# ubc-vision/UniT

Measured on AMD Instinct MI355X. Metric: images/sec (fwd+bwd+SGD) R101-C4 VOC 600x1000 bs=2/GPU, higher is better.
Workload: dtype bf16; 1 GPU; UniT base-training step S1 (TrainerNoMeta.run_step): ResNet-101-C4, VOC split1 K=20, 2 supervised + 2 weak 3x600x1000 images per GPU, 512 RoIs/image, two Res5 heads, RPN 12000->2000, all 8 losses, SGD momentum; images_per_gpu=2, global_batch=2, parallelism=dp1

## Files before the change

include/unit_hip.h:

```cpp
#ifndef UNIT_HIP_H
#define UNIT_HIP_H
#include <stddef.h>
#include <stdint.h>
#ifdef __cplusplus
extern "C" {
#endif

int unit_version(void);
const char* unit_build_hash(void);
const char* unit_last_error(void);

int unit_preprocess_image(const float* img_chw, int C, int H, int W, const float* mean3, const float* std3, float prescale,
                          void* out_nhwc, int out_dtype, int Hmax, int Wmax, int Cpad, void* stream);
int unit_resize_u8_pass(const unsigned char* src, int H, int W, int C, int axis, const int* bounds, const int* kk, int ksize,
                        int out_size, unsigned char* dst, void* stream);
int unit_preprocess_u8(const unsigned char* img_hwc, int C, int H, int W, int hflip, const float* mean3, const float* std3,
                       float prescale, void* out_nhwc, int out_dtype, int Hmax, int Wmax, int Cpad, void* stream);
int unit_image_chw_to_u8(const void* img_chw, int src_u8, int C, int H, int W, unsigned char* out_hwc, void* stream);
int unit_tta_boxes(const float* props, const int* count, int P, int Pcap, const float* views, int V, float* out, void* stream);
int unit_nchw_to_nhwc(const float* x, void* y, int dtype, int N, int C, int H, int W, int Cp, void* stream);
int unit_nhwc_to_nchw(const void* x, int dtype, float* y, int N, int C, int H, int W, int Cp, void* stream);
int unit_debug_spin(long long cycles, void* sink, void* stream);
int unit_cast(const void* x, int in_dtype, void* y, int out_dtype, long n, void* stream);
int unit_fill_zero(void* p, size_t nbytes, void* stream);
int unit_add_cast(const float* a32, const void* b, const void* mask_ref, void* y, int dtype, long n, void* stream);

int unit_conv2d_fwd(const void* x, const void* w, void* y, const float* bias, const void* residual, const void* mask_ref,
                    int in_dtype, int out_dtype, int N, int H, int W, int C, int K, int R, int S, int stride, int pad, int OH,
                    int OW, int ldy, int oy_mul, int OHf, int OWf, int relu, int tile_cfg, void* stream);
int unit_conv2d_fwd_big(const void* x, const void* w, void* y, const float* bias, const void* residual, const void* mask_ref,
                        int out_dtype, int N, int H, int W, int C, int K, int R, int S, int stride, int pad, int OH, int OW, int ldy,
                        int oy_mul, int OHf, int OWf, int relu, int variant, void* stream);
size_t unit_conv_pool_partial_floats(int M, int ldy);
size_t unit_relu_bits_bytes(int M, int ldy);
int unit_conv2d_fwd_big_ex(const void* x, const void* w, void* y, const float* bias, const void* residual, const unsigned char* mask_bits,
                           unsigned char* relu_bits, float* pool_partial, int pool_rows, int N, int H, int W, int C, int K, int R, int S,
                           int pad, int ldy, int relu, const void* x2, int C2, int variant, void* stream);
int unit_pool_finish(const float* partial, int R, int rows, int ldy, int K, void* out, int ldo, int out_dtype, void* stream);
int unit_avgpool_bwd_bits(const void* dfeat, const unsigned char* bits, int R, int roi_offset, int rows, int C, void* g, void* stream);
int unit_conv2d_fwd_mid(const void* x, const void* w, void* y, const float* bias, const void* residual, const void* mask_ref,
                        int out_dtype, int N, int H, int W, int C, int K, int R, int S, int stride, int pad, int OH, int OW, int ldy,
                        int oy_mul, int OHf, int OWf, int relu, int tile, void* stream);
int unit_x3_split(const float* x, void* out, long rows, int C, void* stream);
int unit_x3_merge(const void* in, float* out, long rows, int C, void* stream);
int unit_weight_prep_x3(const float* w_krsc, const float* scale_k, int K, int R, int S, int C, void* w_fwd, void* w_dgrad, void* stream);
int unit_conv2d_fwd_x3(const void* x, const void* w, void* y, const float* bias, const void* residual, const void* mask_ref, int mask_c,
                       int N, int H, int W, int C, int K, int R, int S, int stride, int pad, int OH, int OW, int ldy, int oy_mul, int OHf,
                       int OWf, int relu, int tile, void* stream);
int unit_weight_prep_x3s(const float* w_krsc, const float* scale_k, int K, int R, int S, int C, void* w_fwd, void* w_dgrad, int dgrad_segs,
                         void* stream);
int unit_conv2d_fwd_x3s(const void* x, const void* w, void* y, const float* bias, const void* residual, const void* mask_ref, int mask_c,
                        int N, int H, int W, int C, int K, int R, int S, int stride, int pad, int OH, int OW, int ldy, int oy_mul, int OHf,
                        int OWf, int relu, int tile, int segs, void* stream);
int unit_conv2d_wgrad_x3(const void* x, const void* dy, float* dw, const float* scale_k, int N, int H, int W, int C, int K, int R, int S,
                         int stride, int pad, int OH, int OW, int ldy, int accumulate, int variant, void* workspace, size_t workspace_bytes,
                         void* stream);
int unit_global_avgpool_x3_fwd(const void* y, float* out, int R, int rows, int C, void* stream);
int unit_global_avgpool_x3_bwd_relu(const float* dfeat, const void* y, void* g, int R, int rows, int C, void* stream);
typedef struct UnitConvSecond {
  const void* x; void* y; const void* residual; const void* mask_ref;
  int N, H, W, OHf, OWf;
} UnitConvSecond;
int unit_conv2d_fwd_pair(int kernel, const void* x, const void* w, void* y, const float* bias, const void* residual, const void* mask_ref, int mask_c,
                         int in_dtype, int out_dtype, int N, int H, int W, int C, int K, int R, int S, int stride, int pad, int OH, int OW, int ldy,
                         int oy_mul, int OHf, int OWf, int relu, int tile, const UnitConvSecond* second, void* stream);
size_t unit_conv2d_wgrad_workspace_bytes(int in_dtype, int N, int OH, int OW, int K, int R, int S, int C);
int unit_conv2d_wgrad(const void* x, const void* dy, float* dw, const float* scale_k, int in_dtype, int N, int H, int W, int C,
                      int K, int R, int S, int stride, int pad, int OH, int OW, int ldy, int accumulate, int variant, void* workspace,
                      size_t workspace_bytes, void* stream);
int unit_conv2d_wgrad_splits(int in_dtype, int N, int OH, int OW, int K, int R, int S, int C);
typedef struct UnitWgradProblem {
  const void* x; const void* dy; void* partial;
  int N, H, W, C, K, R, S, stride, pad, OH, OW, ldy;
  int splits, kind;
  int x_pitch;
  int x_back, dy_back;
} UnitWgradProblem;
size_t unit_wgrad_problem_bytes(void);
int unit_conv2d_wgrad_group_supported(int in_dtype, int N, int OH, int OW, int K, int R, int S, int C);
int unit_conv2d_wgrad_group_plan(UnitWgradProblem* pr, int n, int splits_hint);
int unit_conv2d_wgrad_group(const UnitWgradProblem* pr, int n, int in_dtype, void* stream);
int unit_conv2d_wgrad_group_layout(const UnitWgradProblem* pr, int n, int* layout, int layout_rows, int* rows);
int unit_wgrad256_loop(void);
int unit_stream_wait_stream(void* waiter, void* signaller);
size_t unit_tensor_desc_bytes(void);
int unit_multi_wgrad_reduce(const void* descs_dev, int n, int total_blocks, float* grads_flat, void* stream);
int unit_multi_weight_prep(const void* descs_dev, int n, int total_blocks, const float* params_flat, int dtype, void* stream);
int unit_shard_sum(const void* parts, int dtype, int nparts, long n, float* out, void* stream);
int unit_comm_unique_id(void* id, int id_bytes);
int unit_comm_init(int rank, int world, const void* id, int id_bytes, void** comm);
int unit_allreduce_bucket_async(void* comm, void* buf, long count, int dtype, void* stream);
int unit_comm_wait(void* compute_stream, void* comm_stream);
int unit_comm_destroy(void* comm);
int unit_comm_rccl_version(void);
int unit_frozen_bn_fold(const float* w, const float* b, const float* rm, const float* rv, float eps, float* scale, float* shift,
                        int C, void* stream);
int unit_weight_prep(const float* w_krsc, const float* scale_k, int K, int R, int S, int C, int Cp, void* w_fwd, void* w_dgrad,
                     int dtype, void* stream);
size_t unit_bias_grad_scratch_bytes(int M, int K);
int unit_bias_grad(const void* dy, int dtype, int M, int K, int ld, float* db, int accumulate, float* scratch, size_t scratch_bytes,
                   void* stream);
size_t unit_linear_wgrad_workspace_bytes(int R, int C, int K);
int unit_linear_wgrad(const void* x, const void* dy, int dtype, int R, int C, int K, int ldy, float* dw, float* db,
                      void* workspace, size_t workspace_bytes, void* stream);
int unit_stem_conv_pool(const void* x, const void* w, const float* shift, void* y, int dtype, int N, int H, int W, void* stream);
int unit_maxpool3x3s2_fwd(const void* x, void* y, int dtype, int N, int H, int W, int C, void* stream);
int unit_global_avgpool_fwd(const void* x, void* y, int dtype, int R, int P, int C, void* stream);
int unit_global_avgpool_bwd_relu(const void* dfeat, const void* out, void* g, int dtype, int R, int P, int C, void* stream);

int unit_anchor_grid(float* out, int H, int W, int A, float stride, float offset, const float* cell_dev, void* stream);

size_t unit_iou_match_workspace_bytes(int B, int Mcap);
int unit_iou_match(const float* gt, const int* gt_count, int B, int Mcap, const float* boxes, long box_batch_stride,
                   const int* box_count, int Ncap, const float* thresholds, const int* labels, int n_thresh,
                   int allow_low_quality, int64_t* match_idx, int8_t* match_label, float* match_val, void* workspace,
                   size_t workspace_bytes, void* stream);
int unit_pairwise_iou(const float* b1, int M, const float* b2, int Nb, float* out, void* stream);
int unit_match_matrix(const float* q, int M, int N, const float* thresholds, const int* labels, int n_thresh, int allow_low_quality,
                      int64_t* match_idx, int8_t* match_label, float* match_val, float* rowmax_ws, void* stream);

int unit_subsample_labels(const void* labels, int labels_are_int64, const int* count, int B, int Ncap, const int* perm, int Pcap,
                          int num_samples, int max_pos, int bg_label, int8_t* out_labels, int* sampled_idx, int* out_counts,
                          void* stream);

int unit_box_encode(const float* src, const float* tgt, const float* weights4, float* out, int n, void* stream);
int unit_box_decode(const float* deltas, int ld, int col0, int K, const float* boxes, const float* weights4, float scale_clamp,
                    float* out, int n, void* stream);

size_t unit_sort_workspace_bytes(int B, int n);
int unit_sort_desc_stable(const float* src, long batch_stride, int ld, int A, int col0, int B, int n, float* out_keys, int* out_idx,
                          void* workspace, size_t workspace_bytes, void* stream);
int unit_sort_desc_stable_topk(const float* src, long batch_stride, int ld, int A, int col0, int B, int n, int topk,
                               float min_exclusive, float* out_keys, int* out_idx, void* workspace, size_t workspace_bytes,
                               void* stream);
int unit_rpn_decode_select(const float* head, long head_batch_stride, int ld, int A, int delta_col0, const float* anchors,
                           const int* sorted_idx, const float* sorted_logit, int B, int Ncap, int topk, const float* image_hw_dev,
                           float scale_clamp, float min_size, float* cand_boxes, float* cand_scores, int* cand_count, void* stream);
size_t unit_nms_workspace_bytes(int B, int cap);
int unit_nms_max_candidates(void);
int unit_nms(const float* boxes_sorted, const float* scores_sorted, const int* count, int B, int cap, float thresh, int max_keep,
             int* keep_idx, int* keep_count, float* out_boxes, float* out_scores, void* workspace, size_t workspace_bytes,
             void* stream);

int unit_append_gt(const float* props, const int* pcount, int Pcap, const float* gt, const int* gcount, int Mcap, int B, float* cat,
                   int* ccount, void* stream);
int unit_roi_classes(const int64_t* match_idx, const int8_t* match_label, const int* count, const int64_t* gt_classes,
                     const int* gcount, int Mcap, int B, int Ncap, int K, int64_t* cls, void* stream);
int unit_gather_rois(const float* cat, int Ncap, const int* sampled_idx, int S, const int64_t* cls, const int64_t* match_idx,
                     const float* gt, const int* gcount, int Mcap, int B, float* rois, int* roi_cls, float* roi_gt, void* stream);
int unit_first_k_rois(const float* props, const int* pcount, int Pcap, int S, int B, int batch_index_offset, float* rois, int* valid,
                      void* stream);

int unit_roi_align_fwd(const void* feat_nhwc, int dtype, int N, int H, int W, int C, const float* rois, const int* roi_count_dev,
                       int R, int pooled_size, int out_size, int bin_step, float spatial_scale, int sampling_ratio, int aligned,
                       void* out, void* stream);
int unit_roi_align_bwd(const void* gout, int dtype, int N, int H, int W, int C, const float* rois, const int* roi_count_dev, int R,
                       int pooled_size, int out_size, int bin_step, float spatial_scale, int sampling_ratio, int aligned,
                       float* dfeat_f32, void* stream);

size_t unit_roi_align_bwd_gather_workspace_bytes(int R);
int unit_roi_align_bwd_gather(const void* gout, int dtype, int N, int H, int W, int C, const float* rois, const int* roi_count_dev,
                              int R, int rois_per_image, int image_offset, int pooled_size, int out_size, int bin_step,
                              float spatial_scale, int sampling_ratio, int aligned, const void* addend, int addend_images,
                              const void* mask_ref, void* dfeat, int out_dtype, void* workspace, size_t workspace_bytes,
                              void* stream);

size_t unit_rpn_loss_scratch_bytes(int B, int Ncap);
int unit_rpn_loss(const float* head, int ld, int A, int dcol0, const int8_t* labels, const int64_t* match_idx, const float* gt_boxes,
                  int Mcap, const float* anchors, int B, int Ncap, float normalizer, float gscale, float* loss2, void* dhead,
                  int dhead_dtype, float* scratch, size_t scratch_bytes, void* stream);
int unit_rpn_loss_w(const float* head, int ld, int A, int dcol0, const int8_t* labels, const int64_t* match_idx, const float* gt_boxes,
                    int Mcap, const float* anchors, int B, int Ncap, float normalizer, float gscale, float w_cls, float w_loc, float* loss2,
                    void* dhead, int dhead_dtype, float* scratch, size_t scratch_bytes, void* stream);
#define UNIT_BOXLOSS_SMOOTH_L1 0
#define UNIT_BOXLOSS_GIOU 1
int unit_rpn_loss_ex(const float* head, int ld, int A, int dcol0, const int8_t* labels, const int64_t* match_idx, const float* gt_boxes,
                     int Mcap, const float* anchors, int B, int Ncap, float normalizer, float gscale, float w_cls, float w_loc, float* loss2,
                     void* dhead, int dhead_dtype, float* scratch, size_t scratch_bytes, int loss_type, float beta, void* stream);
int unit_sup_scores(const float* delta, int ldd, int dcol0, const float* weak, int ldw, int wcol0, int n_oicr, int ncls,
                    const unsigned char* novel_mask_dev, const float* extra, int lde, int ecol0, float* out, int ldo, int R,
                    void* stream);
int unit_softmax_ce(const float* logits, int ld, int col0, int ncls, const int* labels, const float* weights, int R, float gscale,
                    float* loss, void* dy, int dy_dtype, int ldd, int dcol0, unsigned long long* acc, void* stream);
int unit_box_reg_loss(const float* bbox, int ld, int col0, int K, const int* labels, const float* rois5, const float* gt_boxes,
                      const float* weights4, int R, float gscale, float* loss, void* dy, int dy_dtype, int ldd, int dcol0,
                      unsigned long long* acc, void* stream);
int unit_box_reg_loss_ex(const float* bbox, int ld, int col0, int K, const int* labels, const float* rois5, const float* gt_boxes,
                         const float* weights4, int R, float gscale, float* loss, void* dy, int dy_dtype, int ldd, int dcol0,
                         unsigned long long* acc, int loss_type, float beta, void* stream);
int unit_wsddn_mil(const float* streams, int ld, int ccol0, int dcol0, int K, const int* valid, int S, int B,
                   const unsigned char* multihot, float cls_temp, float det_temp, float mil_multiplier, float gscale, float* loss,
                   float* xr_out, void* dy, int dy_dtype, int ldd, int dyc0, int dyd0, void* stream);
int unit_oicr_targets(const float* src, int ld, int col0, int mode, int K, const float* rois5, const int* valid, int S, int B,
                      const unsigned char* multihot, float fg_thresh, float bg_thresh, int* labels, float* weights, void* stream);
int unit_oicr_targets_ex(const float* src, int ld, int col0, int mode, int K, const float* rois5, const int* valid, int S, int B,
                         const unsigned char* multihot, float fg_thresh, float bg_thresh, int* labels, float* weights, float* gt_boxes,
                         void* stream);
int unit_softmax_mean(const float* logits, int ld, int col0, int step, int n, int K, const int* valid, float* out, int ldo, int R,
                      void* stream);
int unit_sum_losses(const float* losses, int n, float* out, void* stream);
int unit_pcl_loss(const float* logits, int ld, int col0, int K, const int* valid, int S, int B, const int* labels, const float* cls_weights,
                  const int* gt_assign, const int* pc_count, const float* pc_img_cls_weights, const float* pc_probs, const int* n_pc,
                  int ldc, float gscale, float* loss, void* dy, int dy_dtype, int ldd, int dcol0, unsigned long long* acc, void* stream);
size_t unit_workspace_bytes_pcl_targets(int B, int S, int n_streams);
int unit_kmeans_draws(unsigned long long* bits7);
int unit_pcl_targets(const float* src, int ld, int col0, int mode, int step, const float* nxt, int ldn, int ncol0, int nmode, int nstep, int K,
                     const float* rois5, const int* valid, int S, int B, int n_streams, const unsigned char* multihot, float fg_thresh,
                     float bg_thresh, float graph_iou_thresh, int max_pc_num, int* labels, float* cls_weights, int* gt_assign, int* n_pc,
                     int* pc_labels, int* pc_count, float* pc_img_cls_weights, float* pc_probs, int ldc, void* workspace,
                     size_t workspace_bytes, void* stream);
int unit_pcl_targets_ex(const float* src, int ld, int col0, int mode, int step, const float* nxt, int ldn, int ncol0, int nmode, int nstep,
                        int K, const float* rois5, const int* valid, int S, int B, int n_streams, const unsigned char* multihot,
                        float fg_thresh, float bg_thresh, float graph_iou_thresh, int max_pc_num, int* labels, float* cls_weights,
                        int* gt_assign, int* n_pc, int* pc_labels, int* pc_count, float* pc_img_cls_weights, float* pc_probs, int ldc,
                        float* gt_boxes, void* workspace, size_t workspace_bytes, void* stream);
int unit_perm_keys(unsigned long long seed, const long long* counter_dev, int stream_id, int B, int n, float* keys, void* stream);
int unit_counter_bump(long long* counter_dev, long long delta, void* stream);

int unit_embedding_similarity(const float* emb, int ld, int dim, const int* novel_rows, int n_novel, const int* base_rows, int n_base,
                              float* out, void* stream);
int unit_similarity(const float* lin_weak, int ld, int col0, int n_oicr, int ncls, const int* base_dev, int n_base, const float* lingual,
                    int n_novel, float visual_threshold, int use_lingual, int use_visual, float* sim, int R, void* stream);
int unit_transfer_predictions(const float* lin, int ld, int ccol0, int bcol0, int K, const float* weak, int ldw, int wcol0, int n_oicr,
                              const float* ft, int ldf, int fccol0, int fbcol0, const float* sim_cls, const float* sim_bbox,
                              const int* base_dev, int n_base, const int* novel_dev, int n_novel, const int8_t* role_dev,
                              const int* slot_dev, float* scores, int lds, float* bbox, int ldb, int R, void* stream);
int unit_transfer_predictions_ex(const float* lin, int ld, int ccol0, int bcol0, int K, const float* weak, int ldw, int wcol0, int n_oicr,
                                 int wbcol0, const float* ft, int ldf, int fccol0, int fbcol0, const float* sim_cls, const float* sim_bbox,
                                 const int* base_dev, int n_base, const int* novel_dev, int n_novel, const int8_t* role_dev,
                                 const int* slot_dev, float* scores, int lds, float* bbox, int ldb, int R, void* stream);
int unit_transfer_predictions_bwd(const void* dy, int dy_dtype, int ldd, int dccol0, int dbcol0, const float* lin, int ld, int ccol0,
                                  int bcol0, int K, const float* sim_cls, const float* sim_bbox, const int* base_dev, int n_base,
                                  const int* novel_dev, int n_novel, const int8_t* role_dev, const int* slot_dev, void* dlin, int ldl,
                                  float* dsim, int R, void* stream);
int unit_similarity_bwd(const float* lin_weak, int ld, int col0, int n_oicr, int ncls, const int* base_dev, int n_base,
                        const float* lingual, int n_novel, float visual_threshold, int use_lingual, int use_visual, const float* dsim,
                        void* dlin, int dlin_dtype, int ldl, int dcol0, int R, void* stream);
int unit_similarity_static(const float* w_master, int ld, int row0, int n_oicr, int ncls, int D, const int* base_dev, int n_base,
                           const int* novel_dev, int n_novel, const float* lingual, float weight, int use_lingual, int k_topk, int k_wtopk,
                           int k_lsda, float* A, void* stream);
int unit_similarity_ex(const float* lin_weak, int ld, int col0, int n_oicr, int ncls, const int* base_dev, int n_base, const float* A,
                       int n_novel, float visual_threshold, float weight, int use_visual, int k_visual, int average, int none, int product,
                       float* sim, int R, void* stream);
int unit_similarity_bwd_ex(const float* lin_weak, int ld, int col0, int n_oicr, int ncls, const int* base_dev, int n_base, const float* A,
                           int n_novel, float visual_threshold, float weight, int use_visual, int k_visual, int average, int none,
                           int product, const float* dsim, void* dlin, int dlin_dtype, int ldl, int dcol0, int R, void* stream);
int unit_softmax_rows(const float* x, int ld, int ncls, float* y, int ldy, int R, void* stream);
int unit_tta_accumulate(const float* scores, int lds, int scol0, const float* deltas, int ldd, long view_rows, int n_in, int K, int R,
                        const int* count, int v, int n, float* probs_sum, float* delta_sum, float* delta_mean, void* stream);
int unit_detection_candidates(const float* probs, int ldp, const float* deltas, int ldd, const float* props, const int* pcount, int B,
                              int Rcap, int K, const float* weights4, float scale_clamp, const float* image_hw_dev, float score_thresh,
                              int cap, float* cand_boxes, float* cand_scores, int* cand_class, int* cand_roi, int* cand_count,
                              float* cand_max, void* stream);
int unit_detection_offset_gather(const float* cand_boxes, const int* cand_class, const int* order, const int* cand_count,
                                 const float* cand_max, int B, int cap, float* out, void* stream);
int unit_detection_finalize(const float* cand_boxes, const float* cand_scores, const int* cand_class, const int* cand_roi, const int* order,
                            const int* keep, const int* keep_count, int B, int cap, int topk, float* out_boxes, float* out_scores,
                            int* out_class, int* out_roi, int* out_count, void* stream);
int unit_detector_postprocess(float* boxes, const int* count, int B, int topk, const float* scale_xy_dev, const float* out_hw_dev,
                              unsigned char* nonempty, void* stream);
int unit_compact_detections(const float* boxes, const float* scores, const int* cls, const int* roi, const float* masks, int mask_elems,
                            const int* count, const unsigned char* nonempty, int B, int topk, float* oboxes, float* oscores, long* ocls,
                            int* oroi, float* omasks, int* out_count, void* stream);
int unit_boxes_to_rois5(const float* boxes, int B, int T, float* rois5, void* stream);
int unit_gather_rows(const void* src, const int* idx, int B, int T, int rcap, int row_bytes, void* out, void* stream);
int unit_gather_blocks(const void* src, int nb, int block_rows, int take, int row_bytes, void* out, void* stream);
int unit_pseudo_gt(const float* boxes, const float* scores, const int* cls, const int* count, const unsigned char* multihot, int B, int T, int K,
                   float threshold, float* gt_boxes, int* gt_count, int* kept_idx, void* stream);
int unit_gate_anchor_labels(signed char* labels, const int* gt_count, int B, int Ncap, void* stream);

int unit_deconv2x2_weight_prep(const float* w, int Cin, int Cout, void* w_fwd, void* w_dgrad, int dtype, void* stream);
int unit_deconv2x2_grad_unpack(const float* dw_gemm, const float* db_gemm, int Cin, int Cout, float* dw, float* db, void* stream);
int unit_mask_targets(const unsigned char* gt_masks, int Mcap, int Hm, int Wm, const float* rois5, const int* gt_index, const int* cls,
                      int K, int S, int M, unsigned char* out, void* stream);
int unit_mask_targets_polygon(const double* poly_xy, const int* poly_start, const int* inst_start, const int* image_inst0,
                              const float* rois5, const int* gt_index, const int* cls, int K, int S, int M, unsigned char* out, void* stream);
int unit_mask_bce_loss(const float* logits, int K, int ldk, const int* cls, const unsigned char* targets, int S, int M, float gscale,
                       float* loss, void* dlogits, int d_dtype, void* stream);
int unit_mask_bce_loss_ft(const float* logits, int K, int ldk, int delta_col0, const int* cls, const unsigned char* targets,
                          const float* sim, const int* sim_rows, const int* base_dev, int n_base, int n_novel, const int8_t* role_dev,
                          const int* slot_dev, int S, int M, float gscale, float* loss, void* dlogits, int d_dtype, float* dsim,
                          void* stream);
int unit_mask_probs(const float* logits, int K, int ldk, int delta_col0, const int* cls, const float* sim, const int* base_dev, int n_base,
                    int n_novel, const int8_t* role_dev, const int* slot_dev, int S, int M, float* out, void* stream);
int unit_gather_match_index(const int* sampled_idx, int S, const int64_t* match_idx, int Ncap, int B, int* out, void* stream);
int unit_paste_masks(const float* probs, const float* boxes, const unsigned char* valid, int S, int M, int H, int W, float threshold,
                     unsigned char* out, void* stream);

int unit_metrics_rpn(const int8_t* labels, int n, int* m, void* stream);
int unit_metrics_fastrcnn(const float* scores, int ld, int col0, int ncls, const int* roi_cls, int R, int* m, void* stream);
int unit_metrics_mask(const float* logits, int K, int ldk, const int* cls, const unsigned char* targets, int S, int M, int* m, void* stream);

int unit_sgd_momentum(float* p, const float* g, float* buf, long n, float lr, float momentum, float wd, float grad_scale,
                      int first_step, const float* lr_dev, void* stream);

int unit_grad_clip_chunk(void);
size_t unit_grad_clip_workspace_bytes(long g_numel, int n_seg);
int unit_grad_clip_coefs(const float* g, long g_numel, const long* table, int n_seg, int seg_lo, int seg_hi, int n_chunks, int norm_kind,
                         float clip_value, float grad_scale, int full_model, float* norms, float* coefs, void* workspace,
                         size_t workspace_bytes, void* stream);
int unit_sgd_step(float* p, const float* g, float* buf, long lo, long n, float lr, float momentum, float wd, float grad_scale,
                  float clip_value, int first_step, int nesterov, int clip_mode, const long* table, int n_seg, const float* coefs,
                  const float* lr_dev, void* stream);
int unit_sgd_step_masked(float* p, const float* g, float* buf, long lo, long n, float lr, float momentum, float wd, float grad_scale,
                         float clip_value, int first_step, int nesterov, int clip_mode, const long* table, int n_seg, const float* coefs,
                         const unsigned char* live, const float* lr_dev, void* stream);

size_t unit_call_bytes(void);
int unit_replay(const void* calls, int n, int* failed);
int unit_event_record_raw(void* event, void* stream);
int unit_stream_wait_event_raw(void* stream, void* event);
int unit_replay_selftest(int a0, const void* p1, float f0, long a2, int a3, float f1, int a4, int a5, size_t a6, int a7, int a8, float f2,
                         int a9, int a10, int a11, int a12, int a13, int a14, int a15, int a16, int a17, int a18, int a19, int a20,
                         int a21, int a22, int a23, int a24, int a25, int a26, float f3, int a27, long long* out);

#ifdef __cplusplus
}
#endif
#endif
```

unit_amd/csrc/roi_align.hip:

```cpp
#include "common.h"
#include <stdlib.h>

__device__ __forceinline__ long xcd_contiguous(long bid, long n) {
  long q = n / 8, r = n % 8, xcd = bid % 8, loc = bid / 8;
  return (xcd < r ? xcd * (q + 1) : r * (q + 1) + (xcd - r) * q) + loc;
}

struct RoiGeom {
  float sw, sh, bw, bh, count;
  int gh, gw, b;
};

__device__ __forceinline__ RoiGeom roi_geom(const float* __restrict__ roi, float scale, int pooled, int sampling_ratio, bool aligned) {
  RoiGeom g;
  g.b = (int)roi[0];
  float offset = aligned ? 0.5f : 0.0f;
  g.sw = roi[1] * scale - offset; g.sh = roi[2] * scale - offset;
  float ew = roi[3] * scale - offset, eh = roi[4] * scale - offset;
  float rw = ew - g.sw, rh = eh - g.sh;
  if (!aligned) { rw = fmaxf(rw, 1.0f); rh = fmaxf(rh, 1.0f); }
  g.bh = rh / (float)pooled; g.bw = rw / (float)pooled;
  g.gh = sampling_ratio > 0 ? sampling_ratio : (int)ceilf(rh / (float)pooled);
  g.gw = sampling_ratio > 0 ? sampling_ratio : (int)ceilf(rw / (float)pooled);
  g.count = (float)(g.gh * g.gw > 1 ? g.gh * g.gw : 1);
  return g;
}

struct Taps { float w1, w2, w3, w4; int yl, xl, yh, xh; bool valid; };

__device__ __forceinline__ Taps bilinear_taps(float y, float x, int H, int W) {
  Taps t;
  t.valid = !(y < -1.0f || y > (float)H || x < -1.0f || x > (float)W);
  if (y <= 0.f) y = 0.f;
  if (x <= 0.f) x = 0.f;
  int yl = (int)y, xl = (int)x, yh, xh;
  if (yl >= H - 1) { yh = yl = H - 1; y = (float)yl; } else { yh = yl + 1; }
  if (xl >= W - 1) { xh = xl = W - 1; x = (float)xl; } else { xh = xl + 1; }
  float ly = y - (float)yl, lx = x - (float)xl;
  float hy = 1.0f - ly, hx = 1.0f - lx;
  t.w1 = hy * hx; t.w2 = hy * lx; t.w3 = ly * hx; t.w4 = ly * lx;
  t.yl = yl; t.xl = xl; t.yh = yh; t.xh = xh;
  return t;
}

template <typename T, int SR>
__global__ void roi_align_fwd_kernel(const T* __restrict__ feat, int H, int W, int C, const float* __restrict__ rois,
                                     const int* __restrict__ roi_count, int pooled, int out_size, int bin_step, float scale,
                                     int sampling_ratio, int aligned, T* __restrict__ out) {
  int bin = (int)xcd_contiguous(blockIdx.x, gridDim.x);
  int r = bin / (out_size * out_size);
  int pp = bin - r * out_size * out_size;
  int oph = pp / out_size, opw = pp - oph * out_size;
  int c0 = threadIdx.x * 8;
  if (c0 >= C) return;
  T* o = out + ((size_t)bin) * C + c0;
  float acc[8] = {0, 0, 0, 0, 0, 0, 0, 0};
  if (roi_count && r >= *roi_count) { Vec8<T>::store(o, acc); return; }
  RoiGeom g = roi_geom(rois + 5 * (size_t)r, scale, pooled, sampling_ratio, aligned != 0);
  int ph = oph * bin_step, pw = opw * bin_step;
  const T* f = feat + (size_t)g.b * H * W * C + c0;
  if constexpr (SR > 0) {
    Taps t[SR * SR];
    float v[SR * SR][4][8];
#pragma unroll
    for (int iy = 0; iy < SR; ++iy) {
      float y = g.sh + (float)ph * g.bh + ((float)iy + 0.5f) * g.bh / (float)SR;
#pragma unroll
      for (int ix = 0; ix < SR; ++ix) {
        float x = g.sw + (float)pw * g.bw + ((float)ix + 0.5f) * g.bw / (float)SR;
        Taps& q = t[iy * SR + ix];
        q = bilinear_taps(y, x, H, W);
        Vec8<T>::load(f + ((size_t)q.yl * W + q.xl) * C, v[iy * SR + ix][0]);
        Vec8<T>::load(f + ((size_t)q.yl * W + q.xh) * C, v[iy * SR + ix][1]);
        Vec8<T>::load(f + ((size_t)q.yh * W + q.xl) * C, v[iy * SR + ix][2]);
        Vec8<T>::load(f + ((size_t)q.yh * W + q.xh) * C, v[iy * SR + ix][3]);
      }
    }
#pragma unroll
    for (int k = 0; k < SR * SR; ++k) {
      if (!t[k].valid) continue;
#pragma unroll
      for (int i = 0; i < 8; ++i) {
        float val = t[k].w1 * v[k][0][i] + t[k].w2 * v[k][1][i] + t[k].w3 * v[k][2][i] + t[k].w4 * v[k][3][i];
        acc[i] += val;
      }
    }
#pragma unroll
    for (int i = 0; i < 8; ++i) acc[i] = acc[i] / g.count;
    Vec8<T>::store(o, acc);
    return;
  }
  for (int iy = 0; iy < g.gh; ++iy) {
    float y = g.sh + (float)ph * g.bh + ((float)iy + 0.5f) * g.bh / (float)g.gh;
    for (int ix = 0; ix < g.gw; ++ix) {
      float x = g.sw + (float)pw * g.bw + ((float)ix + 0.5f) * g.bw / (float)g.gw;
      Taps t = bilinear_taps(y, x, H, W);
      if (!t.valid) continue;
      float v1[8], v2[8], v3[8], v4[8];
      Vec8<T>::load(f + ((size_t)t.yl * W + t.xl) * C, v1);
      Vec8<T>::load(f + ((size_t)t.yl * W + t.xh) * C, v2);
      Vec8<T>::load(f + ((size_t)t.yh * W + t.xl) * C, v3);
      Vec8<T>::load(f + ((size_t)t.yh * W + t.xh) * C, v4);
#pragma unroll
      for (int i = 0; i < 8; ++i) {
        float val = t.w1 * v1[i] + t.w2 * v2[i] + t.w3 * v3[i] + t.w4 * v4[i];
        acc[i] += val;
      }
    }
  }
#pragma unroll
  for (int i = 0; i < 8; ++i) acc[i] = acc[i] / g.count;
  Vec8<T>::store(o, acc);
}

__device__ __forceinline__ void taps_1d(float v, int n, bool& ok, int& lo, int& hi, float& wlo, float& whi) {
  ok = !(v < -1.0f || v > (float)n);
  if (v <= 0.f) v = 0.f;
  lo = (int)v;
  if (lo >= n - 1) { hi = lo = n - 1; v = (float)lo; } else { hi = lo + 1; }
  whi = v - (float)lo; wlo = 1.0f - whi;
}

template <typename T>
__global__ void __launch_bounds__(256) roi_align_fwd_row_kernel(const T* __restrict__ feat, int H, int W, int C, const float* __restrict__ rois,
                                                                const int* __restrict__ roi_count, int pooled, int out_size, int bin_step,
                                                                float scale, int sampling_ratio, int aligned, T* __restrict__ out) {
  int row = (int)xcd_contiguous(blockIdx.x, gridDim.x);
  int r = row / out_size, oph = row - r * out_size;
  int c0 = threadIdx.x * 8;
  if (c0 >= C) return;
  T* o = out + ((size_t)row * out_size) * C + c0;
  if (roi_count && r >= *roi_count) {
    float z[8] = {0, 0, 0, 0, 0, 0, 0, 0};
    for (int opw = 0; opw < out_size; ++opw) Vec8<T>::store(o + (size_t)opw * C, z);
    return;
  }
  RoiGeom g = roi_geom(rois + 5 * (size_t)r, scale, pooled, sampling_ratio, aligned != 0);
  int ph = oph * bin_step;
  const T* f = feat + (size_t)g.b * H * W * C + c0;
  if (g.gh <= 2 && g.gw <= 2) {
    int rr[4]; float wr[4];
#pragma unroll
    for (int iy = 0; iy < 2; ++iy) {
      float y = g.sh + (float)ph * g.bh + ((float)iy + 0.5f) * g.bh / (float)g.gh;
      bool ok; float wl, wh;
      taps_1d(y, H, ok, rr[2 * iy], rr[2 * iy + 1], wl, wh);
      ok = ok && iy < g.gh;
      wr[2 * iy] = ok ? wl : 0.f; wr[2 * iy + 1] = ok ? wh : 0.f;
    }
#pragma unroll
    for (int k = 1; k < 4; ++k)
#pragma unroll
      for (int j = 0; j < k; ++j)
        if (wr[k] != 0.f && rr[k] == rr[j]) { wr[j] += wr[k]; wr[k] = 0.f; }
    for (int opw = 0; opw < out_size; ++opw) {
      int pw = opw * bin_step;
      int cc[4]; float wc[4];
#pragma unroll
      for (int ix = 0; ix < 2; ++ix) {
        float x = g.sw + (float)pw * g.bw + ((float)ix + 0.5f) * g.bw / (float)g.gw;
        bool ok; float wl, wh;
        taps_1d(x, W, ok, cc[2 * ix], cc[2 * ix + 1], wl, wh);
        ok = ok && ix < g.gw;
        wc[2 * ix] = ok ? wl : 0.f; wc[2 * ix + 1] = ok ? wh : 0.f;
      }
#pragma unroll
      for (int k = 1; k < 4; ++k)
#pragma unroll
        for (int j = 0; j < k; ++j)
          if (wc[k] != 0.f && cc[k] == cc[j]) { wc[j] += wc[k]; wc[k] = 0.f; }
      bf16x8 raw[4][4];
#pragma unroll
      for (int k = 0; k < 4; ++k)
#pragma unroll
        for (int m = 0; m < 4; ++m)
          if (wr[k] != 0.f && wc[m] != 0.f) raw[k][m] = *reinterpret_cast<const bf16x8*>(f + ((size_t)rr[k] * W + cc[m]) * C);
      float acc[8] = {0, 0, 0, 0, 0, 0, 0, 0};
#pragma unroll
      for (int k = 0; k < 4; ++k) {
        if (wr[k] == 0.f) continue;
        float ra[8] = {0, 0, 0, 0, 0, 0, 0, 0};
#pragma unroll
        for (int m = 0; m < 4; ++m) {
          if (wc[m] == 0.f) continue;
#pragma unroll
          for (int i = 0; i < 8; ++i) ra[i] += wc[m] * (float)raw[k][m][i];
        }
#pragma unroll
        for (int i = 0; i < 8; ++i) acc[i] += wr[k] * ra[i];
      }
#pragma unroll
      for (int i = 0; i < 8; ++i) acc[i] = acc[i] / g.count;
      Vec8<T>::store(o + (size_t)opw * C, acc);
    }
    return;
  }
  for (int opw = 0; opw < out_size; ++opw) {
    int pw = opw * bin_step;
    float acc[8] = {0, 0, 0, 0, 0, 0, 0, 0};
    for (int iy = 0; iy < g.gh; ++iy) {
      float y = g.sh + (float)ph * g.bh + ((float)iy + 0.5f) * g.bh / (float)g.gh;
      for (int ix = 0; ix < g.gw; ++ix) {
        float x = g.sw + (float)pw * g.bw + ((float)ix + 0.5f) * g.bw / (float)g.gw;
        Taps t = bilinear_taps(y, x, H, W);
        if (!t.valid) continue;
        float v1[8], v2[8], v3[8], v4[8];
        Vec8<T>::load(f + ((size_t)t.yl * W + t.xl) * C, v1);
        Vec8<T>::load(f + ((size_t)t.yl * W + t.xh) * C, v2);
        Vec8<T>::load(f + ((size_t)t.yh * W + t.xl) * C, v3);
        Vec8<T>::load(f + ((size_t)t.yh * W + t.xh) * C, v4);
#pragma unroll
        for (int i = 0; i < 8; ++i) {
          float val = t.w1 * v1[i] + t.w2 * v2[i] + t.w3 * v3[i] + t.w4 * v4[i];
          acc[i] += val;
        }
      }
    }
#pragma unroll
    for (int i = 0; i < 8; ++i) acc[i] = acc[i] / g.count;
    Vec8<T>::store(o + (size_t)opw * C, acc);
  }
}

extern "C" int unit_roi_align_fwd(const void* feat_nhwc, int dtype, int N, int H, int W, int C, const float* rois,
                                  const int* roi_count_dev, int R, int pooled_size, int out_size, int bin_step,
                                  float spatial_scale, int sampling_ratio, int aligned, void* out, void* stream) {
  (void)N;
  UNIT_CHECK_ARG(C % 8 == 0 && C / 8 <= 1024, "roi_align: C % 8 != 0 or C > 8192");
  UNIT_CHECK_ARG((out_size - 1) * bin_step < pooled_size, "roi_align: out_size/bin_step exceed pooled_size");
  if (R == 0) return UNIT_OK;
  int threads = ((C / 8 + 63) / 64) * 64;
  long blocks = (long)R * out_size * out_size;
  hipStream_t st = (hipStream_t)stream;
  if (dtype == UNIT_BF16 && threads <= 256) {
    roi_align_fwd_row_kernel<bf16_t><<<(long)R * out_size, threads, 0, st>>>((const bf16_t*)feat_nhwc, H, W, C, rois, roi_count_dev, pooled_size, out_size,
                                                                           bin_step, spatial_scale, sampling_ratio, aligned, (bf16_t*)out);
    UNIT_LAUNCH_CHECK();
    return UNIT_OK;
  }
  if (dtype == UNIT_BF16 && sampling_ratio == 2)
    roi_align_fwd_kernel<bf16_t, 2><<<blocks, threads, 0, st>>>((const bf16_t*)feat_nhwc, H, W, C, rois, roi_count_dev, pooled_size, out_size, bin_step,
                                                              spatial_scale, sampling_ratio, aligned, (bf16_t*)out);
  else if (dtype == UNIT_BF16)
    roi_align_fwd_kernel<bf16_t, 0><<<blocks, threads, 0, st>>>((const bf16_t*)feat_nhwc, H, W, C, rois, roi_count_dev, pooled_size, out_size, bin_step,
                                                              spatial_scale, sampling_ratio, aligned, (bf16_t*)out);
  else
    roi_align_fwd_kernel<float, 0><<<blocks, threads, 0, st>>>((const float*)feat_nhwc, H, W, C, rois, roi_count_dev, pooled_size, out_size, bin_step,
                                                             spatial_scale, sampling_ratio, aligned, (float*)out);
  UNIT_LAUNCH_CHECK();
  return UNIT_OK;
}

template <typename T>
__global__ void roi_align_bwd_kernel(const T* __restrict__ gout, int H, int W, int C, const float* __restrict__ rois,
                                     const int* __restrict__ roi_count, int pooled, int out_size, int bin_step, float scale,
                                     int sampling_ratio, int aligned, float* __restrict__ dfeat) {
  int bin = blockIdx.x;
  int r = bin / (out_size * out_size);
  int pp = bin - r * out_size * out_size;
  int oph = pp / out_size, opw = pp - oph * out_size;
  if (roi_count && r >= *roi_count) return;
  RoiGeom g = roi_geom(rois + 5 * (size_t)r, scale, pooled, sampling_ratio, aligned != 0);
  int ph = oph * bin_step, pw = opw * bin_step;
  float* d = dfeat + (size_t)g.b * H * W * C;
  const T* go = gout + (size_t)bin * C;
  for (int c = threadIdx.x; c < C; c += blockDim.x) {
    float gg = (float)go[c];
    for (int iy = 0; iy < g.gh; ++iy) {
      float y = g.sh + (float)ph * g.bh + ((float)iy + 0.5f) * g.bh / (float)g.gh;
      for (int ix = 0; ix < g.gw; ++ix) {
        float x = g.sw + (float)pw * g.bw + ((float)ix + 0.5f) * g.bw / (float)g.gw;
        Taps t = bilinear_taps(y, x, H, W);
        if (!t.valid) continue;
        atomicAdd(d + ((size_t)t.yl * W + t.xl) * C + c, gg * t.w1 / g.count);
        atomicAdd(d + ((size_t)t.yl * W + t.xh) * C + c, gg * t.w2 / g.count);
        atomicAdd(d + ((size_t)t.yh * W + t.xl) * C + c, gg * t.w3 / g.count);
        atomicAdd(d + ((size_t)t.yh * W + t.xh) * C + c, gg * t.w4 / g.count);
      }
    }
  }
}

extern "C" int unit_roi_align_bwd(const void* gout, int dtype, int N, int H, int W, int C, const float* rois,
                                  const int* roi_count_dev, int R, int pooled_size, int out_size, int bin_step,
                                  float spatial_scale, int sampling_ratio, int aligned, float* dfeat_f32, void* stream) {
  (void)N;
  if (R == 0) return UNIT_OK;
  int threads = C >= 256 ? 256 : ((C + 63) / 64) * 64;
  long blocks = (long)R * out_size * out_size;
  hipStream_t st = (hipStream_t)stream;
  if (dtype == UNIT_BF16)
    roi_align_bwd_kernel<bf16_t><<<blocks, threads, 0, st>>>((const bf16_t*)gout, H, W, C, rois, roi_count_dev, pooled_size, out_size, bin_step,
                                                           spatial_scale, sampling_ratio, aligned, dfeat_f32);
  else
    roi_align_bwd_kernel<float><<<blocks, threads, 0, st>>>((const float*)gout, H, W, C, rois, roi_count_dev, pooled_size, out_size, bin_step,
                                                          spatial_scale, sampling_ratio, aligned, dfeat_f32);
  UNIT_LAUNCH_CHECK();
  return UNIT_OK;
}

struct RoiG { float sw, sh, bw, bh, inv_count; int gh, gw, b, y0, y1, x0, x1; };

__global__ void roi_geom_kernel(const float* __restrict__ rois, const int* __restrict__ roi_count, int R, int H, int W, int pooled,
                                int out_size, int bin_step, float scale, int sampling_ratio, int aligned, RoiG* __restrict__ tab) {
  int r = blockIdx.x * blockDim.x + threadIdx.x;
  if (r >= R) return;
  RoiG t;
  if (roi_count && r >= *roi_count) { t.b = -1; t.y0 = 1; t.y1 = 0; t.x0 = 1; t.x1 = 0; t.gh = t.gw = 0; t.sw = t.sh = t.bw = t.bh = t.inv_count = 0.f; tab[r] = t; return; }
  RoiGeom g = roi_geom(rois + 5 * (size_t)r, scale, pooled, sampling_ratio, aligned != 0);
  t.sw = g.sw; t.sh = g.sh; t.bw = g.bw; t.bh = g.bh; t.inv_count = 1.0f / g.count; t.gh = g.gh; t.gw = g.gw; t.b = g.b;
  int plast = (out_size - 1) * bin_step;
  if (g.gh <= 0 || g.gw <= 0) { t.y0 = 1; t.y1 = 0; t.x0 = 1; t.x1 = 0; }
  else {
    float yf = g.sh + 0.5f * g.bh / (float)g.gh, yl = g.sh + (float)plast * g.bh + ((float)g.gh - 0.5f) * g.bh / (float)g.gh;
    float xf = g.sw + 0.5f * g.bw / (float)g.gw, xl = g.sw + (float)plast * g.bw + ((float)g.gw - 0.5f) * g.bw / (float)g.gw;
    t.y0 = max(0, (int)floorf(fminf(yf, yl)) - 1); t.y1 = min(H - 1, (int)floorf(fmaxf(yf, yl)) + 2);
    t.x0 = max(0, (int)floorf(fminf(xf, xl)) - 1); t.x1 = min(W - 1, (int)floorf(fmaxf(xf, xl)) + 2);
  }
  tab[r] = t;
}

__device__ __forceinline__ float tap1d(float s, int p, int L) {
  if (s < -1.0f || s > (float)L) return 0.f;
  if (s <= 0.f) s = 0.f;
  int lo = (int)s, hi;
  if (lo >= L - 1) { hi = lo = L - 1; s = (float)lo; } else hi = lo + 1;
  float l = s - (float)lo, h = 1.0f - l;
  return (lo == p ? h : 0.f) + (hi == p ? l : 0.f);
}

template <typename T, typename TOUT>
__global__ void roi_align_bwd_gather_kernel(const T* __restrict__ gout, int H, int W, int C, const RoiG* __restrict__ tab, int R,
                                            int rois_per_image, int image_offset, int out_size, int bin_step,
                                            const T* __restrict__ addend, int addend_images, const T* __restrict__ mask_ref,
                                            TOUT* __restrict__ dfeat) {
  extern __shared__ float wlds[];
  int pix = (int)xcd_contiguous(blockIdx.x, gridDim.x);
  int n = pix / (H * W); int rem = pix - n * H * W; int py = rem / W, px = rem - py * W;
  int lane = threadIdx.x & 63, wave = threadIdx.x >> 6;
  float* wy_s = wlds + wave * 32; float* wx_s = wy_s + 16;
  int c0 = threadIdx.x * 8;
  bool cvalid = c0 < C;
  float acc[8] = {0, 0, 0, 0, 0, 0, 0, 0};
  int r_begin = 0, r_end = R;
  if (rois_per_image > 0) { r_begin = n * rois_per_image; r_end = min(R, r_begin + rois_per_image); }
  for (int rb = r_begin; rb < r_end; rb += 64) {
    bool hit = false;
    if (rb + lane < r_end) {
      const RoiG& q = tab[rb + lane];
      hit = q.b == n + image_offset && py >= q.y0 && py <= q.y1 && px >= q.x0 && px <= q.x1;
    }
    for (unsigned long long hm = __ballot(hit); hm; hm &= hm - 1) {
      int r = rb + __ffsll((long long)hm) - 1;
      RoiG t = tab[r];
      float wv = 0.f;
      int o = lane & 31;
      if (o < out_size) {
        bool isx = lane >= 32;
        int p = o * bin_step;
        float start = isx ? t.sw : t.sh, bsz = isx ? t.bw : t.bh;
        int gn = isx ? t.gw : t.gh; int L = isx ? W : H; int pp = isx ? px : py;
        for (int i = 0; i < gn; ++i) {
          float s = start + (float)p * bsz + ((float)i + 0.5f) * bsz / (float)gn;
          wv += tap1d(s, pp, L);
        }
      }
      unsigned long long nz = __ballot(wv != 0.f);
      unsigned ymask = (unsigned)(nz & 0xFFFFFFFFull), xmask = (unsigned)(nz >> 32);
      if (ymask == 0u || xmask == 0u) continue;
      if (o < out_size) { if (lane < 32) wy_s[o] = wv; else wx_s[o] = wv; }
      __builtin_amdgcn_wave_barrier();
      if (cvalid) {
        const T* gr = gout + (size_t)r * out_size * out_size * C + c0;
        for (unsigned ym = ymask; ym; ym &= ym - 1) {
          int oy = __ffs(ym) - 1;
          float wy = wy_s[oy] * t.inv_count;
          for (unsigned xm = xmask; xm; xm &= xm - 1) {
            int ox = __ffs(xm) - 1;
            float w = wy * wx_s[ox];
            float v[8];
            Vec8<T>::load(gr + ((size_t)oy * out_size + ox) * C, v);
#pragma unroll
            for (int j = 0; j < 8; ++j) acc[j] += w * v[j];
          }
        }
      }
      __builtin_amdgcn_wave_barrier();
    }
  }
  if (!cvalid) return;
  size_t o = (size_t)pix * C + c0;
  if (addend && n < addend_images) {
    float a[8]; Vec8<T>::load(addend + o, a);
#pragma unroll
    for (int j = 0; j < 8; ++j) acc[j] += a[j];
  }
  if (mask_ref) {
    float m[8]; Vec8<T>::load(mask_ref + o, m);
#pragma unroll
    for (int j = 0; j < 8; ++j) acc[j] = m[j] > 0.f ? acc[j] : 0.f;
  }
  Vec8<TOUT>::store(dfeat + o, acc);
}

extern "C" size_t unit_roi_align_bwd_gather_workspace_bytes(int R) { return sizeof(RoiG) * (size_t)(R > 0 ? R : 1); }

extern "C" int unit_roi_align_bwd_gather(const void* gout, int dtype, int N, int H, int W, int C, const float* rois,
                                         const int* roi_count_dev, int R, int rois_per_image, int image_offset, int pooled_size, int out_size,
                                         int bin_step, float spatial_scale, int sampling_ratio, int aligned, const void* addend,
                                         int addend_images, const void* mask_ref, void* dfeat, int out_dtype, void* workspace,
                                         size_t workspace_bytes, void* stream) {
  UNIT_CHECK_ARG(C % 8 == 0 && C / 8 <= 1024 && out_size <= 16, "roi_align_bwd_gather: C % 8, C <= 8192, out_size <= 16");
  UNIT_CHECK_ARG(out_dtype == UNIT_F32 || out_dtype == dtype, "roi_align_bwd_gather: out dtype must be fp32 or the input dtype");
  if (workspace_bytes < unit_roi_align_bwd_gather_workspace_bytes(R)) { unit_set_error("roi_align_bwd_gather: workspace too small"); return UNIT_ERR_WORKSPACE; }
  hipStream_t st = (hipStream_t)stream;
  RoiG* tab = (RoiG*)workspace;
  if (R > 0) {
    roi_geom_kernel<<<cdiv(R, 256), 256, 0, st>>>(rois, roi_count_dev, R, H, W, pooled_size, out_size, bin_step, spatial_scale,
                                                sampling_ratio, aligned, tab);
    UNIT_LAUNCH_CHECK();
  }
  int threads = ((C / 8 + 63) / 64) * 64;
  size_t lds = (size_t)(threads / 64) * 32 * sizeof(float);
  long blocks = (long)N * H * W;
  if (blocks == 0) return UNIT_OK;
#define LAUNCH_G(T, TOUT) roi_align_bwd_gather_kernel<T, TOUT><<<blocks, threads, lds, st>>>((const T*)gout, H, W, C, tab, R, rois_per_image, \
    image_offset, out_size, bin_step, (const T*)addend, addend_images, (const T*)mask_ref, (TOUT*)dfeat)
  if (dtype == UNIT_BF16 && out_dtype == UNIT_BF16) LAUNCH_G(bf16_t, bf16_t);
  else if (dtype == UNIT_BF16) LAUNCH_G(bf16_t, float);
  else LAUNCH_G(float, float);
#undef LAUNCH_G
  UNIT_LAUNCH_CHECK();
  return UNIT_OK;
}
```

Before: 135.7 images/sec.

## Restructure RoIAlign backward gather into cooperative tap list with pipelined loads

Replaces the per-pixel RoIAlign backward gather kernel with a version where up to two waves test RoI hits and compute separable per-axis bilinear weights together. They build a compact LDS list of nonzero (output-bin index, weight) taps via ballots and prefix scans. All channel threads then stream through that list with double-buffered, unrolled vector loads, which aims to hide gather latency and skip zero-weight bins. The old kernel is kept as a reference entry point. The cost is more LDS per block, extra block-wide barriers and more complex code, which may reduce occupancy.

Result: no change. 135.4 images/sec (-0.2%).

```diff
diff --git a/include/unit_hip.h b/include/unit_hip.h
--- a/include/unit_hip.h
+++ b/include/unit_hip.h
@@ -164,6 +164,11 @@
                               float spatial_scale, int sampling_ratio, int aligned, const void* addend, int addend_images,
                               const void* mask_ref, void* dfeat, int out_dtype, void* workspace, size_t workspace_bytes,
                               void* stream);
+int unit_roi_align_bwd_gather_ref(const void* gout, int dtype, int N, int H, int W, int C, const float* rois, const int* roi_count_dev,
+                                  int R, int rois_per_image, int image_offset, int pooled_size, int out_size, int bin_step,
+                                  float spatial_scale, int sampling_ratio, int aligned, const void* addend, int addend_images,
+                                  const void* mask_ref, void* dfeat, int out_dtype, void* workspace, size_t workspace_bytes,
+                                  void* stream);
 
 size_t unit_rpn_loss_scratch_bytes(int B, int Ncap);
 int unit_rpn_loss(const float* head, int ld, int A, int dcol0, const int8_t* labels, const int64_t* match_idx, const float* gt_boxes,
diff --git a/unit_amd/csrc/roi_align.hip b/unit_amd/csrc/roi_align.hip
--- a/unit_amd/csrc/roi_align.hip
+++ b/unit_amd/csrc/roi_align.hip
@@ -330,7 +330,7 @@
 }
 
 template <typename T, typename TOUT>
-__global__ void roi_align_bwd_gather_kernel(const T* __restrict__ gout, int H, int W, int C, const RoiG* __restrict__ tab, int R,
+__global__ void roi_align_bwd_gather_ref_kernel(const T* __restrict__ gout, int H, int W, int C, const RoiG* __restrict__ tab, int R,
                                             int rois_per_image, int image_offset, int out_size, int bin_step,
                                             const T* __restrict__ addend, int addend_images, const T* __restrict__ mask_ref,
                                             TOUT* __restrict__ dfeat) {
@@ -403,13 +403,226 @@
   Vec8<TOUT>::store(dfeat + o, acc);
 }
 
+#define GB_NB 2
+#define GB_TCAP 512
+
+template <typename T> struct Raw8;
+template <> struct Raw8<bf16_t> {
+  bf16x8 a;
+  __device__ __forceinline__ void load(const bf16_t* p) { a = *reinterpret_cast<const bf16x8*>(p); }
+  __device__ __forceinline__ float get(int i) const { return (float)a[i]; }
+};
+template <> struct Raw8<float> {
+  f32x4 a, b;
+  __device__ __forceinline__ void load(const float* p) { a = *reinterpret_cast<const f32x4*>(p); b = *reinterpret_cast<const f32x4*>(p + 4); }
+  __device__ __forceinline__ float get(int i) const { return i < 4 ? a[i] : b[i - 4]; }
+};
+
+template <typename T, int U>
+__device__ __forceinline__ void gb_issue(const T* __restrict__ g0, int C, const i32x2* taps, int t, int last, Raw8<T> (&raw)[U], float (&w)[U]) {
+#pragma unroll
+  for (int k = 0; k < U; ++k) {
+    i32x2 e = taps[min(t + k, last)];
+    w[k] = __int_as_float(e[1]);
+    raw[k].load(g0 + (size_t)e[0] * C);
+  }
+}
+
+template <typename T, int U>
+__device__ __forceinline__ void gb_fma(const Raw8<T> (&raw)[U], const float (&w)[U], float (&acc)[8]) {
+#pragma unroll
+  for (int k = 0; k < U; ++k)
+#pragma unroll
+    for (int j = 0; j < 8; ++j) acc[j] += w[k] * raw[k].get(j);
+}
+
+static size_t gb_lds_bytes(int threads, int out_size) {
+  int nb = threads / 64 < GB_NB ? threads / 64 : GB_NB;
+  int lph = out_size <= 8 ? 16 : 32;
+  return (size_t)GB_TCAP * 8 + 8 * 4 + (size_t)nb * 64 * (8 + 1 + lph + 1) * 4;
+}
+
+template <typename T, typename TOUT>
+__global__ void roi_align_bwd_gather_kernel(const T* __restrict__ gout, int H, int W, int C, const RoiG* __restrict__ tab, int R,
+                                            int rois_per_image, int image_offset, int out_size, int bin_step,
+                                            const T* __restrict__ addend, int addend_images, const T* __restrict__ mask_ref,
+                                            TOUT* __restrict__ dfeat) {
+  constexpr int U = sizeof(T) == 2 ? 4 : 2;
+  extern __shared__ __attribute__((aligned(16))) unsigned char gb_lds[];
+  const int lane = threadIdx.x & 63, wave = threadIdx.x >> 6, nw = blockDim.x >> 6;
+  const int nb = nw < GB_NB ? nw : GB_NB;
+  const int sh = out_size <= 8 ? 3 : 4, S = 1 << sh, LPH = 2 << sh, WS = LPH + 1;
+  i32x2* taps = reinterpret_cast<i32x2*>(gb_lds);
+  int* tot = reinterpret_cast<int*>(taps + GB_TCAP);
+  float* seg = reinterpret_cast<float*>(tot + 8) + (size_t)(wave < nb ? wave : 0) * 64 * (9 + WS);
+  float* rec = seg;
+  float* msk = seg + 64 * 8;
+  float* wts = msk + 64;
+  int pix = (int)xcd_contiguous(blockIdx.x, gridDim.x);
+  int n = pix / (H * W); int rem = pix - n * H * W; int py = rem / W, px = rem - py * W;
+  int c0 = threadIdx.x * 8;
+  bool cvalid = c0 < C;
+  const T* g0 = gout + (cvalid ? c0 : 0);
+  const int oo = out_size * out_size;
+  float acc[8] = {0, 0, 0, 0, 0, 0, 0, 0};
+  int r_begin = 0, r_end = R;
+  if (rois_per_image > 0) { r_begin = n * rois_per_image; r_end = min(R, r_begin + rois_per_image); }
+  int par = 0;
+  for (int rb0 = r_begin; rb0 < r_end; rb0 += 64 * nb, par ^= 4) {
+    int nh = 0, my_off = 0, my_r = 0, my_nt = 0;
+    unsigned my_mask = 0u;
+    if (wave < nb) {
+      int r = rb0 + 64 * wave + lane;
+      bool hit = false;
+      RoiG q;
+      if (r < r_end) {
+        q = tab[r];
+        hit = q.b == n + image_offset && py >= q.y0 && py <= q.y1 && px >= q.x0 && px <= q.x1;
+      }
+      unsigned long long hm = __ballot(hit);
+      nh = __popcll(hm);
+      if (hit) {
+        float* rc = rec + 8 * __popcll(hm & ((1ull << lane) - 1ull));
+        rc[0] = q.sw; rc[1] = q.sh; rc[2] = q.bw; rc[3] = q.bh; rc[4] = q.inv_count;
+        rc[5] = __int_as_float(q.gh); rc[6] = __int_as_float(q.gw); rc[7] = __int_as_float(r);
+      }
+      __builtin_amdgcn_wave_barrier();
+      for (int h0 = 0; h0 < nh; h0 += 64 >> (sh + 1)) {
+        int hs = lane >> (sh + 1), h = h0 + hs, li = lane & (LPH - 1);
+        bool isx = li >= S;
+        int o = li & (S - 1);
+        bool live = h < nh && o < out_size;
+        float wv = 0.f, inv = 0.f;
+        if (live) {
+          const float* rc = rec + 8 * h;
+          float start = rc[isx ? 0 : 1], bsz = rc[isx ? 2 : 3];
+          int gn = __float_as_int(rc[isx ? 6 : 5]);
+          inv = rc[4];
+          int L = isx ? W : H, pp = isx ? px : py, p = o * bin_step;
+          for (int i = 0; i < gn; ++i) {
+            float s = start + (float)p * bsz + ((float)i + 0.5f) * bsz / (float)gn;
+            wv += tap1d(s, pp, L);
+          }
+        }
+        unsigned long long nz = __ballot(wv != 0.f);
+        if (live) wts[h * WS + li] = isx ? wv : wv * inv;
+        if (h < nh && li == 0) {
+          unsigned m = (unsigned)(nz >> (hs * LPH));
+          unsigned ym = m & ((1u << S) - 1u), xm = (m >> S) & ((1u << S) - 1u);
+          msk[h] = __uint_as_float(ym | (xm << 16));
+        }
+      }
+      __builtin_amdgcn_wave_barrier();
+      if (lane < nh) { my_mask = __float_as_uint(msk[lane]); my_r = __float_as_int(rec[8 * lane + 7]); }
+      int ntl = __popc(my_mask & 0xFFFFu) * __popc(my_mask >> 16);
+      int inc = ntl;
+#pragma unroll
+      for (int d = 1; d < 64; d <<= 1) {
+        int v = __shfl_up(inc, d, 64);
+        if (lane >= d) inc += v;
+      }
+      my_off = inc - ntl; my_nt = ntl;
+      int total = __shfl(inc, 63, 64);
+      if (lane == 0) tot[par + wave] = total;
+    }
+    __syncthreads();
+    int base = 0, tall = 0;
+    for (int i = 0; i < nb; ++i) { int v = tot[par + i]; if (i < wave) base += v; tall += v; }
+    for (int win0 = 0; win0 < tall; win0 += GB_TCAP) {
+      if (wave < nb) {
+        int p = base + my_off - win0;
+        if (my_nt > 0 && p < GB_TCAP && p + my_nt > 0) {
+          const float* wh = wts + lane * WS;
+          int e0 = my_r * oo;
+          for (unsigned ym = my_mask & 0xFFFFu; ym; ym &= ym - 1u) {
+            int oy = __ffs(ym) - 1;
+            float wy = wh[oy];
+            for (unsigned xm = my_mask >> 16; xm; xm &= xm - 1u) {
+              int ox = __ffs(xm) - 1;
+              if (p >= 0 && p < GB_TCAP) {
+                i32x2 e;
+                e[0] = e0 + oy * out_size + ox;
+                e[1] = __float_as_int(wy * wh[S + ox]);
+                taps[p] = e;
+              }
+              ++p;
+            }
+          }
+        }
+      }
+      __syncthreads();
+      int nt = min(GB_TCAP, tall - win0);
+      if (cvalid) {
+        int nbat = (nt + U - 1) / U, full = nt / U, last = nt - 1;
+        Raw8<T> ra[U], rb[U];
+        float wa[U], wb[U];
+        gb_issue<T, U>(g0, C, taps, 0, last, ra, wa);
+        int b = 1;
+        while (b + 1 < full) {
+          gb_issue<T, U>(g0, C, taps, b * U, last, rb, wb);
+          gb_fma<T, U>(ra, wa, acc);
+          gb_issue<T, U>(g0, C, taps, (b + 1) * U, last, ra, wa);
+          gb_fma<T, U>(rb, wb, acc);
+          b += 2;
+        }
+        if (b < nbat) gb_issue<T, U>(g0, C, taps, b * U, last, rb, wb);
+        if (b - 1 < full) gb_fma<T, U>(ra, wa, acc);
+        else {
+#pragma unroll
+          for (int k = 0; k < U; ++k)
+            if ((b - 1) * U + k < nt) {
+#pragma unroll
+              for (int j = 0; j < 8; ++j) acc[j] += wa[k] * ra[k].get(j);
+            }
+        }
+        if (b < nbat) {
+          if (b < full) gb_fma<T, U>(rb, wb, acc);
+          else {
+#pragma unroll
+            for (int k = 0; k < U; ++k)
+              if (b * U + k < nt) {
+#pragma unroll
+                for (int j = 0; j < 8; ++j) acc[j] += wb[k] * rb[k].get(j);
+              }
+          }
+          ++b;
+        }
+        if (b < nbat) {
+          gb_issue<T, U>(g0, C, taps, b * U, last, ra, wa);
+#pragma unroll
+          for (int k = 0; k < U; ++k)
+            if (b * U + k < nt) {
+#pragma unroll
+              for (int j = 0; j < 8; ++j) acc[j] += wa[k] * ra[k].get(j);
+            }
+        }
+      }
+      __syncthreads();
+    }
+  }
+  if (!cvalid) return;
+  size_t o = (size_t)pix * C + c0;
+  if (addend && n < addend_images) {
+    float a[8]; Vec8<T>::load(addend + o, a);
+#pragma unroll
+    for (int j = 0; j < 8; ++j) acc[j] += a[j];
+  }
+  if (mask_ref) {
+    float m[8]; Vec8<T>::load(mask_ref + o, m);
+#pragma unroll
+    for (int j = 0; j < 8; ++j) acc[j] = m[j] > 0.f ? acc[j] : 0.f;
+  }
+  Vec8<TOUT>::store(dfeat + o, acc);
+}
+
+
 extern "C" size_t unit_roi_align_bwd_gather_workspace_bytes(int R) { return sizeof(RoiG) * (size_t)(R > 0 ? R : 1); }
 
-extern "C" int unit_roi_align_bwd_gather(const void* gout, int dtype, int N, int H, int W, int C, const float* rois,
-                                         const int* roi_count_dev, int R, int rois_per_image, int image_offset, int pooled_size, int out_size,
-                                         int bin_step, float spatial_scale, int sampling_ratio, int aligned, const void* addend,
-                                         int addend_images, const void* mask_ref, void* dfeat, int out_dtype, void* workspace,
-                                         size_t workspace_bytes, void* stream) {
+static int roi_align_bwd_gather_launch(bool ref, const void* gout, int dtype, int N, int H, int W, int C, const float* rois,
+                                       const int* roi_count_dev, int R, int rois_per_image, int image_offset, int pooled_size, int out_size,
+                                       int bin_step, float spatial_scale, int sampling_ratio, int aligned, const void* addend,
+                                       int addend_images, const void* mask_ref, void* dfeat, int out_dtype, void* workspace,
+                                       size_t workspace_bytes, void* stream) {
   UNIT_CHECK_ARG(C % 8 == 0 && C / 8 <= 1024 && out_size <= 16, "roi_align_bwd_gather: C % 8, C <= 8192, out_size <= 16");
   UNIT_CHECK_ARG(out_dtype == UNIT_F32 || out_dtype == dtype, "roi_align_bwd_gather: out dtype must be fp32 or the input dtype");
   if (workspace_bytes < unit_roi_align_bwd_gather_workspace_bytes(R)) { unit_set_error("roi_align_bwd_gather: workspace too small"); return UNIT_ERR_WORKSPACE; }
@@ -421,15 +634,39 @@
     UNIT_LAUNCH_CHECK();
   }
   int threads = ((C / 8 + 63) / 64) * 64;
-  size_t lds = (size_t)(threads / 64) * 32 * sizeof(float);
+  size_t lds = ref ? (size_t)(threads / 64) * 32 * sizeof(float) : gb_lds_bytes(threads, out_size);
   long blocks = (long)N * H * W;
   if (blocks == 0) return UNIT_OK;
-#define LAUNCH_G(T, TOUT) roi_align_bwd_gather_kernel<T, TOUT><<<blocks, threads, lds, st>>>((const T*)gout, H, W, C, tab, R, rois_per_image, \
+#define LAUNCH_G(K, T, TOUT) K<T, TOUT><<<blocks, threads, lds, st>>>((const T*)gout, H, W, C, tab, R, rois_per_image, \
     image_offset, out_size, bin_step, (const T*)addend, addend_images, (const T*)mask_ref, (TOUT*)dfeat)
-  if (dtype == UNIT_BF16 && out_dtype == UNIT_BF16) LAUNCH_G(bf16_t, bf16_t);
-  else if (dtype == UNIT_BF16) LAUNCH_G(bf16_t, float);
-  else LAUNCH_G(float, float);
+#define LAUNCH_GK(K) do { \
+    if (dtype == UNIT_BF16 && out_dtype == UNIT_BF16) LAUNCH_G(K, bf16_t, bf16_t); \
+    else if (dtype == UNIT_BF16) LAUNCH_G(K, bf16_t, float); \
+    else LAUNCH_G(K, float, float); } while (0)
+  if (ref) LAUNCH_GK(roi_align_bwd_gather_ref_kernel);
+  else LAUNCH_GK(roi_align_bwd_gather_kernel);
+#undef LAUNCH_GK
 #undef LAUNCH_G
   UNIT_LAUNCH_CHECK();
   return UNIT_OK;
 }
+
+extern "C" int unit_roi_align_bwd_gather(const void* gout, int dtype, int N, int H, int W, int C, const float* rois,
+                                         const int* roi_count_dev, int R, int rois_per_image, int image_offset, int pooled_size, int out_size,
+                                         int bin_step, float spatial_scale, int sampling_ratio, int aligned, const void* addend,
+                                         int addend_images, const void* mask_ref, void* dfeat, int out_dtype, void* workspace,
+                                         size_t workspace_bytes, void* stream) {
+  return roi_align_bwd_gather_launch(false, gout, dtype, N, H, W, C, rois, roi_count_dev, R, rois_per_image, image_offset, pooled_size, out_size,
+                                     bin_step, spatial_scale, sampling_ratio, aligned, addend, addend_images, mask_ref, dfeat, out_dtype,
+                                     workspace, workspace_bytes, stream);
+}
+
+extern "C" int unit_roi_align_bwd_gather_ref(const void* gout, int dtype, int N, int H, int W, int C, const float* rois,
+                                             const int* roi_count_dev, int R, int rois_per_image, int image_offset, int pooled_size,
+                                             int out_size, int bin_step, float spatial_scale, int sampling_ratio, int aligned,
+                                             const void* addend, int addend_images, const void* mask_ref, void* dfeat, int out_dtype,
+                                             void* workspace, size_t workspace_bytes, void* stream) {
+  return roi_align_bwd_gather_launch(true, gout, dtype, N, H, W, C, rois, roi_count_dev, R, rois_per_image, image_offset, pooled_size, out_size,
+                                     bin_step, spatial_scale, sampling_ratio, aligned, addend, addend_images, mask_ref, dfeat, out_dtype,
+                                     workspace, workspace_bytes, stream);
+}
```
